# adolliou/euispice_coreg

Hardware: AMD Instinct MI355X
Metric: lag-points/sec (whole node) on 2048² grid, 60×60 CRVAL sweep; argmax-shift match (higher is better)
Workload: dtype f64; 1 GPU; headline: Carrington 'fa' 2048x2048 grid lon(200,300) lat(-20,20), 60x60 CRVAL lags arange(-30,30,1) arcsec, small 2048^2 HRIEUV-like, ref 3072^2 FSI-like, order 2, solar_r 1.004; lag_points=3600, parallelism=single GPU, no collective, resident=True, sweeps_in_flight=2, small_stored_f32=True, use_lds=True

## Files before the change

### euispice_coreg_amd/csrc/coreg_hip.hip

```cpp
#include <hip/hip_runtime.h>

#include <algorithm>
#include <chrono>
#include <cmath>
#include <cstdio>
#include <cstdlib>
#include <cstring>
#include <limits>
#include <condition_variable>
#include <map>
#include <memory>
#include <mutex>
#include <string>
#include <thread>
#include <functional>
#include <type_traits>
#include <utility>
#include <vector>

#include "fit.hpp"
#include "geometry.hpp"
#include "kernels.hpp"
#include <atomic>
#include "ricecomp.hpp"
#include "riceenc.hpp"

using namespace coreg;

#define COREG_VERSION "0.1.0"

#include "lag_plan.hpp"
#include "sweep_plan.hpp"
#include "host_owned.hpp"
#include "host_state.hpp"
#include "host_upload.hpp"
#include "host_smooth.hpp"
#include "host_plan.hpp"
#include "host_fix_launch.hpp"
#include "sweep_variant.hpp"
#include "host_sweep_launch.hpp"
#include "host_sweep_mi.hpp"
#include "host_fix_lists.hpp"
#include "host_sweep_io.hpp"
#include "host_context.hpp"
#include "pixels_plan.hpp"
#include "host_pixels.hpp"

coreg_handle::~coreg_handle() = default;

extern "C" {

const char* coreg_version(void) { return "coreg_hip " COREG_VERSION " (gfx950)"; }

int coreg_create(coreg_handle** out, int device) {
    if (!out) return COREG_EINVAL;
    *out = nullptr;
    int ndev = 0;
    hipError_t e = hipGetDeviceCount(&ndev);
    if (e != hipSuccess || ndev < 1) return COREG_EHIP;
    if (device < 0) {
        if (hipGetDevice(&device) != hipSuccess) device = 0;
    }
    if (device >= ndev) return COREG_EINVAL;
    coreg_handle* h = new (std::nothrow) coreg_handle();
    if (!h) return COREG_ENOMEM;
    h->device = device;
    if (hipSetDevice(device) != hipSuccess || hipStreamCreateWithFlags(&h->stream.s, hipStreamNonBlocking) != hipSuccess ||
        hipEventCreate(&h->ev_end[0].e) != hipSuccess ||
        hipEventCreate(&h->ev_end[1].e) != hipSuccess || hipEventRecord(h->ev_end[0], h->stream) != hipSuccess ||
        hipEventRecord(h->ev_end[1], h->stream) != hipSuccess ||
        h->pivots.reserve(2 * sizeof(double)) != hipSuccess ||
        hipMemsetAsync(h->pivots.p, 0, 2 * sizeof(double), h->stream) != hipSuccess) {
        coreg_destroy(h);
        return COREG_EHIP;
    }
    std::memset(&h->stats, 0, sizeof(h->stats));
    *out = h;
    return COREG_OK;
}

void coreg_destroy(coreg_handle* h) {
    if (!h) return;
    (void)hipSetDevice(h->device);
    if (h->up_thread.joinable()) {
        {
            std::unique_lock<std::mutex> lk(h->up_m);
            h->up_cv.wait(lk, [&] { return !h->up_busy && !h->up_has; });
            h->up_stop = true;
        }
        h->up_cv.notify_all();
        h->up_thread.join();
    }
    if (h->stream) (void)hipStreamSynchronize(h->stream);
    if (h->up_stream) (void)hipStreamSynchronize(h->up_stream);
    delete h;
}

const char* coreg_last_error(const coreg_handle* h) { return h ? h->err.c_str() : "null handle"; }

int coreg_set_stream(coreg_handle* h, void* hip_stream) {
    if (!h) return COREG_EINVAL;
    RETCHK(bind_device(h));
    RETCHK(collect_stats(h));
    HIPCHK(hipStreamSynchronize(h->stream));
    HIPCHK(h->stream.borrow((hipStream_t)hip_stream));
    return COREG_OK;
}

int coreg_synchronize(coreg_handle* h) {
    if (!h) return COREG_EINVAL;
    RETCHK(bind_device(h));
    HIPCHK(hipStreamSynchronize(h->stream));
    return COREG_OK;
}

int coreg_set_option(coreg_handle* h, const char* name, int64_t value) {
    if (!h || !name) return COREG_EINVAL;
    const std::string n(name);
    if (n == "use_lds") {
        h->opt_use_lds = value ? 1 : 0;
    } else if (n == "clean_path") {
        h->opt_clean_path = value ? 1 : 0;
    } else if (n == "tap_nan_filter") {
        if (value < 0 || value > 2) return fail(h, COREG_EINVAL, "tap_nan_filter must be 0, 1 or 2");
        h->opt_tap_nan_filter = value;
    } else if (n == "overlap_upload") {
        h->opt_overlap_upload = value ? 1 : 0;
    } else if (n == "async_upload") {
        h->opt_async_upload = value ? 1 : 0;
    } else if (n == "refine") {
        h->opt_refine = value ? 1 : 0;
    } else if (n == "refine_cond_log10") {
        if (value < -3 || value > 15) return fail(h, COREG_EINVAL, "refine_cond_log10 must be in [-3, 15]");
        h->opt_refine_cond_log10 = value;
    } else if (n == "refine_max") {
        if (value < 0 || value > 16) return fail(h, COREG_EINVAL, "refine_max must be in [0, 16]");
    } else if (n == "tile_w") {
        if (value != 0 && (value < 1 || value > kTilePts || (value & (value - 1)) != 0))
            return fail(h, COREG_EINVAL, "tile_w must be 0 or a power of two <= 1024");
        h->opt_tile_w = value;
    } else if (n == "n_groups") {
        if (value < 0) return fail(h, COREG_EINVAL, "n_groups must be >= 0");
        h->opt_n_groups = value;
    } else if (n == "sweep_wgs") {
        if (value < 0) return fail(h, COREG_EINVAL, "sweep_wgs must be >= 0");
        h->opt_sweep_wgs = value;
    } else if (n == "skew") {
        (void)value;
    } else if (n == "shard_world") {
        if (value < 1 || value > 64) return fail(h, COREG_EINVAL, "shard_world must be in [1, 64]");
        h->opt_shard_world = value;
        if (h->opt_shard_rank >= value) h->opt_shard_rank = 0;
    } else if (n == "combo_begin") {
        if (value < 0) return fail(h, COREG_EINVAL, "combo_begin must be >= 0");
        h->opt_combo_begin = value;
    } else if (n == "combo_end") {
        if (value < 0) return fail(h, COREG_EINVAL, "combo_end must be >= 0");
        h->opt_combo_end = value;
    } else if (n == "shard_rank") {
        if (value < 0 || value >= h->opt_shard_world) return fail(h, COREG_EINVAL, "shard_rank must be in [0, shard_world)");
        h->opt_shard_rank = value;
    } else if (n == "border_fix") {
        h->opt_border_fix = value ? 1 : 0;
    } else if (n == "tap_fix") {
        h->opt_tap_fix = value ? 1 : 0;
    } else if (n == "tap_cap") {
        if (value < 1 || value > (1 << 26)) return fail(h, COREG_EINVAL, "tap_cap must be in [1, 2^26]");
        h->opt_tap_cap = value;
    } else if (n == "pitch") {
        h->opt_pitch = value;
    } else if (n == "taper_frac") {
        if (value < -1 || value > 1000) return fail(h, COREG_EINVAL, "taper_frac must be in [-1, 1000]");
        h->opt_taper_frac = value;
    } else if (n == "taper_min") {
        if (value < 16 || value > 1024) return fail(h, COREG_EINVAL, "taper_min must be in [16, 1024]");
        h->opt_taper_min = value;
    } else if (n == "taper_rounds") {
        if (value < 1) return fail(h, COREG_EINVAL, "taper_rounds must be >= 1");
        h->opt_taper_rounds = value;
    } else if (n == "crop_reference") {
        h->opt_crop_reference = value ? 1 : 0;
    } else if (n == "tile_skip") {
        h->opt_tile_skip = value ? 1 : 0;
    } else if (n == "h_series") {
        h->opt_h_series = value ? 1 : 0;
    } else if (n == "h_incr") {
        h->opt_h_incr = value ? 1 : 0;
    } else if (n == "patch_w") {
        if (value < 0 || value > kBlock) return fail(h, COREG_EINVAL, "patch_w must be in [0, 256]");
        h->opt_patch_w = value;
    } else if (n == "mi_chunks") {
        if (value < 0 || value > kMiMaxChunks) return fail(h, COREG_EINVAL, "mi_chunks must be in [0, 64]");
        h->opt_mi_chunks = value;
    } else if (n == "lds_bytes") {
        if (value < 1024 || value > 159 * 1024) return fail(h, COREG_EINVAL, "lds_bytes must be in [1 KiB, 159 KiB]");
        h->opt_lds_bytes = value;
    } else {
        return fail(h, COREG_EINVAL, "unknown option: " + n);
    }
    return COREG_OK;
}

}

#include "abi_images.hpp"
#include "abi_sweeps.hpp"
#include "abi_host.hpp"
#include "abi_context.hpp"
#include "abi_pixels.hpp"


#include "multi.hpp"
```

### euispice_coreg_amd/csrc/host_plan.hpp

```cpp
#pragma once
namespace {

struct ComboRange {
    long long begin = 0, end = 0;
};
ComboRange take_combo_range(coreg_handle* h) {
    ComboRange r;
    r.begin = h->opt_combo_begin;
    r.end = h->opt_combo_end;
    h->opt_combo_begin = h->opt_combo_end = 0;
    return r;
}
int check_lags(coreg_handle* h, const coreg_lags* l, LagDims* d, int64_t begin, int64_t end, ComboRange combo = ComboRange()) {
    if (!l || !l->crval1 || !l->crval2 || !l->cdelt1 || !l->cdelt2 || !l->crota)
        return fail(h, COREG_EINVAL, "lags: null array");
    if (l->n_crval1 < 1 || l->n_crval2 < 1 || l->n_cdelt1 < 1 || l->n_cdelt2 < 1 || l->n_crota < 1)
        return fail(h, COREG_EINVAL, "lags: every axis needs at least one value");
    d->n1 = l->n_crval1;
    d->n2 = l->n_crval2;
    d->n3 = l->n_cdelt1;
    d->n4 = l->n_cdelt2;
    d->n5 = l->n_crota;
    d->nc = (long long)d->n3 * d->n4 * d->n5;
    d->c0 = 0;
    {
        const long long cb = combo.begin, ce = combo.end;
        if (cb != 0 || ce != 0) {
            if (cb < 0 || ce <= cb || ce > d->nc)
                return fail(h, COREG_EINVAL, "combo_begin/combo_end outside [0, n_cdelt1 * n_cdelt2 * n_crota]");
            d->c0 = cb;
            d->nc = ce - cb;
        }
    }
    if (begin < 0 || end > d->total() || begin > end)
        return fail(h, COREG_EINVAL, "lag_begin/lag_end outside [0, n_lags]");
    const double* ax[5] = {l->crval1, l->crval2, l->cdelt1, l->cdelt2, l->crota};
    const int32_t na[5] = {l->n_crval1, l->n_crval2, l->n_cdelt1, l->n_cdelt2, l->n_crota};
    for (int k = 0; k < 5; ++k)
        for (int32_t i = 0; i < na[k]; ++i)
            if (!std::isfinite(ax[k][i])) return fail(h, COREG_EINVAL, "lags: a non-finite value");
    return COREG_OK;
}

static int check_wcs(coreg_handle* h, const coreg_wcs2d* w, bool carrington_transform) {
    const char* why = wcs_problem(*w, carrington_transform);
    return why ? fail(h, COREG_EINVAL, why) : COREG_OK;
}
static int check_grid(coreg_handle* h, const coreg_carr_grid* g) {
    if (g->n_lon >= 1 && g->n_lat >= 1 && too_many(g->n_lon, g->n_lat))
        return fail(h, COREG_EINVAL, "Carrington grid: more than 2^31 - 1 points");
    const char* why = grid_problem(*g);
    return why ? fail(h, COREG_EINVAL, why) : COREG_OK;
}

int pick_groups(const coreg_handle* h, int n_batches, int n_tiles) {
    (void)n_tiles;
    return coreg::pick_groups(h->opt_shard_world, h->opt_n_groups, n_batches);
}

long long lds_window_elems(const coreg_handle* h);
SweepEnv sweep_env(coreg_handle* h) {
    SweepEnv e;
    e.sW = h->sW;
    e.sH = h->sH;
    e.gW = h->gW;
    e.gH = h->gH;
    e.border_fix = h->opt_border_fix != 0;
    e.tap_fix = h->opt_tap_fix != 0;
    e.use_lds = h->opt_use_lds != 0;
    e.h_series = h->opt_h_series != 0;
    e.tile_skip = h->opt_tile_skip != 0;
    e.lds_elems = lds_window_elems(h);
    e.tile_w = (int)h->opt_tile_w;
    e.patch_w = (int)h->opt_patch_w;
    e.shard_world = h->opt_shard_world;
    e.n_groups = h->opt_n_groups;
    e.pitch = h->opt_pitch;
    e.tabs = &h->tabs;
    e.caches = &h->wcslib;
    e.memo = &h->plan_memo;
    return e;
}

void pick_taper(const coreg_handle* h, int n_groups, int n_batches, int* tmin, int* tfrac) {
    *tmin = (int)h->opt_taper_min;
    if (h->opt_taper_frac >= 0) {
        *tfrac = (int)h->opt_taper_frac;
        return;
    }
    const double rounds = (double)n_groups * n_batches / 256.0;
    *tfrac = (rounds >= (double)h->opt_taper_rounds && n_groups >= 128 && h->opt_shard_world <= 1) ? 512 : 0;
}

template <int MODE>
int launch_precompute(coreg_handle* h, const PrecomputeArgs& a, int n_tiles, int n_groups, int n_batches) {
    EventPair* ev = next_event(h, h->ev_pre, h->ev_pre_used);
    if (!ev) return fail(h, COREG_EHIP, "hipEventCreate failed");
    int tmin, tfrac;
    pick_taper(h, n_groups, n_batches, &tmin, &tfrac);
    PrecomputeArgs b = a;
    b.prologue = h->pending_prologue;
    const bool with_prologue = b.prologue.src != nullptr;
    std::memset(&h->pending_prologue, 0, sizeof(h->pending_prologue));
    HIPCHK(hipEventRecord(ev->a, h->stream));
    if (h->ref_dtype == COREG_F32)
        hipLaunchKernelGGL((k_precompute<MODE, float>), dim3(n_tiles), dim3(256), 0, h->stream, b);
    else
        hipLaunchKernelGGL((k_precompute<MODE, double>), dim3(n_tiles), dim3(256), 0, h->stream, b);
    (void)with_prologue;
    hipLaunchKernelGGL(k_tile_list, dim3(1), dim3(1024), 0, h->stream, (const int*)a.tile_count, n_tiles, n_groups,
                       h->tile_list.as<int>(), h->tile_cum.as<int>(), h->group_first.as<int>(),
                       h->tile_info.as<long long>(), tmin, tfrac, (const double*)a.tile_bbox,
                       h->visit_rec.as<VisitRec>());
    ev->b_is_next_sweep = true;
    ev->next_sweep_index = h->ev_sweep_used;
    HIPCHK(hipGetLastError());
    return COREG_OK;
}

int reserve_tiles(coreg_handle* h, int n_tiles) {
    const size_t pts = (size_t)n_tiles * kTilePts + (size_t)(kPointGroups + 1) * kChunk;
    HIPCHK(h->pts.reserve(pts * sizeof(Pt)));
    HIPCHK(h->tile_count.reserve(n_tiles * sizeof(int)));
    HIPCHK(h->tile_list.reserve(n_tiles * sizeof(int)));
    HIPCHK(h->tile_cum.reserve((n_tiles + 1) * sizeof(int)));
    HIPCHK(h->group_first.reserve(2 * 1024 * sizeof(int) + 64));
    HIPCHK(h->tile_info.reserve(8 * sizeof(long long)));
    HIPCHK(h->tile_bbox.reserve((size_t)n_tiles * 4 * sizeof(double)));
    HIPCHK(h->visit_rec.reserve(((size_t)n_tiles + 1) * sizeof(VisitRec)));
    return COREG_OK;
}

int setup_precompute(coreg_handle* h, const Plan& plan, int method, PrecomputeArgs* a, int* n_tiles) {
    std::memset(a, 0, sizeof(*a));
    a->tile_w = plan.tile_w;
    a->tile_h = kTilePts / plan.tile_w;
    a->tiles_x = (h->gW + a->tile_w - 1) / a->tile_w;
    a->tiles_y = (h->gH + a->tile_h - 1) / a->tile_h;
    *n_tiles = a->tiles_x * a->tiles_y;
    RETCHK(reserve_tiles(h, *n_tiles));
    a->ref = h->ref.p;
    a->gw = h->gW;
    a->gh = h->gH;
    a->pivot_a = h->pivots.as<double>();
    a->pts = h->pts.as<Pt>();
    a->tile_count = h->tile_count.as<int>();
    a->tile_bbox = h->tile_bbox.as<double>();
    a->residus = method != COREG_METHOD_CORRELATION ? 1 : 0;
    return COREG_OK;
}

}
```

### euispice_coreg_amd/csrc/host_state.hpp

```cpp
#pragma once
namespace {

enum SrcKind {
    SRC_HOST = 0,
    SRC_PINNED = 1,
    SRC_DEVICE = 2,
    SRC_TILED = 3,
};

struct PixFmt {
    int bitpix = 0;
    bool f32 = false;
    double bscale = 1.0, bzero = 0.0;
    bool raw() const { return bitpix != 0; }
    bool scaled() const { return bscale != 1.0 || bzero != 0.0; }
    size_t elem() const { return raw() ? (size_t)(bitpix < 0 ? -bitpix : bitpix) / 8 : (f32 ? 4 : 8); }
    bool swap_only() const { return bitpix == -32 && !scaled(); }
    static PixFmt native(bool is_f32) {
        PixFmt f;
        f.f32 = is_f32;
        return f;
    }
};

constexpr int kMaxDevices = 64;
std::mutex g_attr_mutex;

struct EventPair {
    Event a, b;
    bool b_is_next_sweep = false;
    size_t next_sweep_index = 0;
};

}

struct KeptTapLists {
    DevBuf all;
};
struct TapFix {
    TapFixArgs args = {};
    int segs = 0;
    int mode = 0;
    long long count = 0;
};
struct FixLaunch {
    std::vector<BorderFixArgs> border;
    std::vector<ParityFixArgs> parity;
    TapFix tap;
    std::shared_ptr<KeptTapLists> kept;
    bool small_f32 = true;
    bool empty() const { return border.empty() && parity.empty() && tap.segs == 0; }
};

struct ContextState;
struct PixelsState;

struct coreg_handle {
    int device = 0;
    Stream stream;
    std::string err;

    std::unique_ptr<ContextState> ctx;
    std::unique_ptr<PixelsState> pix;
    ~coreg_handle();

    DevBuf small;
    int sW = 0, sH = 0;
    bool small_f32 = false;
    DevBuf ref;
    int gW = 0, gH = 0;
    int ref_dtype = -1;
    DevBuf pivots, red_sum, red_cnt;
    DevBuf t_sin_lon, t_cos_lon, t_cos_lat, t_sin_lat, t_lon_deg, t_dx;
    coreg_diffrot rot_ref = {}, rot_small = {};
    bool has_rot_ref = false, has_rot_small = false;
    DevBuf sm_num, sm_den, sm_out;
    std::vector<double> ref_smooth_y, ref_smooth_x;
    CarrTables tabs;
    std::vector<double> tabs_key;
    bool tabs_uploaded = false;
    PinBuf pin_img[2];
    Event ev_img[2];
    int pin_img_next = 0;
    DevBuf pts, tile_count, tile_list, tile_cum, group_first, tile_info, tile_bbox;
    DevBuf visit_rec;
    DevBuf rf_fix_slab;
    DevBuf counters;
    DevBuf lane_params, out_index, partials, out_dev, tmp_img;
    DevBuf sweep_queue;
    int n_cus = 0;
    struct SweepResidency {
        const void* fn;
        size_t lds_bytes;
        int per_cu;
    };
    std::vector<SweepResidency> sweep_residency;
    int64_t opt_sweep_wgs = 0;
    DevBuf counts;
    long long counts_n = -1;
    DevBuf up_f64, up_flag;
    DevBuf up_raw;
    DevBuf rice_blob, rice_rand, dec_img;
    PrologueArgs pending_prologue = {};
    DevBuf bbox_buf;
    Stream aux_stream;
    Stream up_stream;
    Event ev_small, ev_main;
    bool small_pending = false;
    DevBuf red_sum_up, red_cnt_up;
    int64_t opt_overlap_upload = 1;
    int64_t opt_tap_nan_filter = 2;
    int64_t opt_async_upload = 0;
    std::thread up_thread;
    std::mutex up_m;
    std::condition_variable up_cv;
    std::function<hipError_t()> up_job;
    bool up_has = false, up_stop = false, up_busy = false;
    hipError_t up_rc = hipSuccess;
    PinBuf pin_small[2];
    Event ev_pin_small[2];
    int pin_small_next = 0;
    WcslibCaches wcslib;
    DevBuf border_flags, fix_partial;
    DevBuf border_dev;
    PinBuf pin_border;
    int64_t opt_border_fix = 1;
    int64_t opt_tap_fix = 1, opt_tap_cap = 1 << 24;
    DevBuf tap_count, tap_segq, tap_list, tap_skip, tap_seg_slot, tap_seg_begin, tap_pixel, tap_xw, tap_yw;
    long long tap_last[3] = {0, 0, 0};
    int last_variant[7] = {-1, 0, 0, 0, 0, 0, 0};
    int64_t opt_shard_world = 1, opt_shard_rank = 0;
    int64_t opt_combo_begin = 0, opt_combo_end = 0;
    DevBuf sums;
    long long sums_slots = 0;
    struct PendingFinalize {
        long long slot_off, n_slots, lag_begin;
        int residus;
        RefineArgs refine;
        std::function<int(coreg_handle*)> replay_precompute;
        FixLaunch fixes;
    };
    std::function<int(coreg_handle*)> last_precompute;
    PlanMemo plan_memo;
    DevBuf rf_flags, rf_pivots, rf_list, rf_head, rf_partial;
    std::vector<PendingFinalize> pending_fin;
    DevBuf fin_outidx;
    long long pending_n_out = 0;
    std::vector<double> mi_edges_small, mi_edges_large;
    DevBuf mi_hist;
    size_t mi_lds[6] = {0, 0, 0, 0, 0, 0};
    int64_t opt_mi_chunks = 0;

    int64_t opt_crop_reference = 1;
    int64_t opt_taper_min = 128, opt_taper_frac = -1, opt_taper_rounds = 6;
    int64_t opt_use_lds = 1, opt_clean_path = 1, opt_refine = 1, opt_refine_cond_log10 = 5, opt_tile_w = 0, opt_n_groups = 0, opt_lds_bytes = (159 * 1024 * kPointGroups) / 4, opt_patch_w = 0, opt_h_series = 1, opt_h_incr = 1, opt_tile_skip = 1, opt_pitch = -1;

    coreg_stats stats;
    bool stats_pending = false;
    PinBuf pin_info;
    std::vector<EventPair> ev_sweep, ev_pre;
    size_t ev_sweep_used = 0, ev_pre_used = 0;
    hipEvent_t ev_t1 = nullptr;
    Event ev_end[2];
    PinBuf pin_plan[2];
    int plan_slot = 0;
    bool plan_open = false;
};
```

### euispice_coreg_amd/csrc/kernels_prepare.hpp

```cpp
#pragma once
namespace coreg {
template <typename T>
__global__ void __launch_bounds__(256) k_sum_finite(const T* __restrict__ v, long long n, double* part_sum,
                                                    long long* part_cnt) {
    __shared__ double ss[256];
    __shared__ long long sc[256];
    double s = 0.0;
    long long c = 0;
    for (long long i = (long long)blockIdx.x * 256 + threadIdx.x; i < n; i += (long long)gridDim.x * 256) {
        const double x = (double)v[i];
        if (isfinite(x)) {
            s += x;
            ++c;
        }
    }
    ss[threadIdx.x] = s;
    sc[threadIdx.x] = c;
    __syncthreads();
    for (int o = 128; o > 0; o >>= 1) {
        if ((int)threadIdx.x < o) {
            ss[threadIdx.x] += ss[threadIdx.x + o];
            sc[threadIdx.x] += sc[threadIdx.x + o];
        }
        __syncthreads();
    }
    if (threadIdx.x == 0) {
        part_sum[blockIdx.x] = ss[0];
        part_cnt[blockIdx.x] = sc[0];
    }
}
__global__ void k_mean_final(const double* part_sum, const long long* part_cnt, int n, double* mean_out) {
    if (threadIdx.x == 0 && blockIdx.x == 0) {
        double s = 0.0;
        long long c = 0;
        for (int i = 0; i < n; ++i) {
            s += part_sum[i];
            c += part_cnt[i];
        }
        mean_out[0] = c > 0 ? s / (double)c : 0.0;
    }
}

__global__ void __launch_bounds__(256) k_f32_exact(const double* __restrict__ v, long long n, int* flag) {
    int bad = 0;
    for (long long i = (long long)blockIdx.x * 256 + threadIdx.x; i < n; i += (long long)gridDim.x * 256) {
        const double x = v[i];
        if (x == x && (double)(float)x != x) bad = 1;
    }
    if (bad) atomicOr(flag, 1);
}
__global__ void __launch_bounds__(256) k_f64_to_f32(const double* __restrict__ v, long long n, float* __restrict__ out) {
    for (long long i = (long long)blockIdx.x * 256 + threadIdx.x; i < n; i += (long long)gridDim.x * 256)
        out[i] = (float)v[i];
}

__global__ void __launch_bounds__(256) k_fits_swap32(unsigned int* __restrict__ v, long long n) {
    for (long long i = (long long)blockIdx.x * 256 + threadIdx.x; i < n; i += (long long)gridDim.x * 256)
        v[i] = __builtin_bswap32(v[i]);
}
__global__ void __launch_bounds__(256) k_fits_to_f64(const void* __restrict__ raw, int bitpix, int scaled, double bscale,
                                                     double bzero, long long n, double* __restrict__ out) {
#pragma clang fp contract(off)
    for (long long i = (long long)blockIdx.x * 256 + threadIdx.x; i < n; i += (long long)gridDim.x * 256) {
        double x;
        switch (bitpix) {
            case 8: x = (double)((const unsigned char*)raw)[i]; break;
            case 16: x = (double)(short)__builtin_bswap16(((const unsigned short*)raw)[i]); break;
            case 32: x = (double)(int)__builtin_bswap32(((const unsigned int*)raw)[i]); break;
            case 64: x = (double)(long long)__builtin_bswap64(((const unsigned long long*)raw)[i]); break;
            case -32: x = (double)__uint_as_float(__builtin_bswap32(((const unsigned int*)raw)[i])); break;
            default: x = __longlong_as_double((long long)__builtin_bswap64(((const unsigned long long*)raw)[i])); break;
        }
        if (scaled) x = x * bscale + bzero;
        out[i] = x;
    }
}

template <typename T>
__global__ void __launch_bounds__(256) k_threshold(T* __restrict__ v, long long n, int has_min, double vmin, int has_max,
                                                   double vmax) {
    for (long long i = (long long)blockIdx.x * 256 + threadIdx.x; i < n; i += (long long)gridDim.x * 256) {
        const double x = fabs((double)v[i]);
        if ((has_min && x < vmin) || (has_max && x > vmax)) v[i] = (T)__builtin_nan("");
    }
}

__global__ void k_fill(double* p, long long n, double v) {
    const long long i = (long long)blockIdx.x * blockDim.x + threadIdx.x;
    if (i < n) p[i] = v;
}

struct ResampleArgs {
    const void* img;
    int W, H;
    int gw, gh;
    CarrDev carr;
    double x0, y0;
    H9 hom;
    void* out;
    int order_rt;
    Crop crop;
    double* bbox;
    LaunchU car_fwd, car_inv;
};
template <int MODE>
__device__ __forceinline__ bool resample_coord(const ResampleArgs& a, long long idx, double& nx, double& ny) {
    const int i = (int)(idx % a.gw), j = (int)(idx / a.gw);
    bool ok = true;
    if (MODE == MODE_TRANSLATE) {
        double t0, t1;
        ok = carr_term(a.carr, i, j, t0, t1);
        nx = a.x0 + t0;
        ny = a.y0 + t1;
    } else if (MODE == MODE_CAR) {
        const double phi = fma(a.car_fwd.m00, (double)i, fma(a.car_fwd.m01, (double)j, a.car_fwd.b0));
        const double theta = fma(a.car_fwd.m10, (double)i, fma(a.car_fwd.m11, (double)j, a.car_fwd.b1));
        apply_car(a.hom, a.car_inv, phi, theta, nx, ny);
    } else {
        apply_h(a.hom, (double)i, (double)j, nx, ny);
    }
    if (!ok) nx = __builtin_nan("");
    return (nx >= 0.0) & (nx <= (double)(a.W - 1)) & (ny >= 0.0) & (ny <= (double)(a.H - 1));
}
template <int MODE>
__global__ void __launch_bounds__(256) k_resample_bbox(const ResampleArgs a) {
    __shared__ double red[4][4];
    const double inf = __builtin_inf();
    double mnx = inf, mxx = -inf, mny = inf, mxy = -inf;
    const long long n = (long long)a.gw * a.gh;
    for (long long idx = (long long)blockIdx.x * 256 + threadIdx.x; idx < n; idx += (long long)gridDim.x * 256) {
        double nx, ny;
        if (resample_coord<MODE>(a, idx, nx, ny)) {
            mnx = fmin(mnx, nx);
            mxx = fmax(mxx, nx);
            mny = fmin(mny, ny);
            mxy = fmax(mxy, ny);
        }
    }
    for (int o = 32; o > 0; o >>= 1) {
        mnx = fmin(mnx, __shfl_xor(mnx, o));
        mxx = fmax(mxx, __shfl_xor(mxx, o));
        mny = fmin(mny, __shfl_xor(mny, o));
        mxy = fmax(mxy, __shfl_xor(mxy, o));
    }
    const int lane = threadIdx.x & 63, wave = threadIdx.x >> 6;
    if (lane == 0) {
        red[wave][0] = mnx;
        red[wave][1] = mxx;
        red[wave][2] = mny;
        red[wave][3] = mxy;
    }
    __syncthreads();
    if (threadIdx.x == 0) {
// ... 39 lines not shown
    for (long long i = i0; i < p.n_outidx; i += stride) p.dst_outidx[i] = src_idx[i];
    const double nan = __builtin_nan("");
    for (long long i = i0; i < p.n_out; i += stride) p.out[i] = nan;
    if (p.counts)
        for (long long i = i0; i < p.n_out; i += stride) p.counts[i] = nan;
}

struct PrecomputeArgs {
    PrologueArgs prologue;
    const void* ref;
    int gw, gh;
    int tile_w, tile_h;
    int tiles_x, tiles_y;
    CarrDev carr;
    LaunchU car_fwd;
    double f0lo, f0hi, f1lo, f1hi;
    int residus;
    int tile_skip;
    double lip_x, lip_y;
    double dlon, dlat;
    const double* pivot_a;
    Pt* pts;
    int* tile_count;
    double* tile_bbox;
};
template <int MODE, typename TA>
__global__ void __launch_bounds__(256) k_precompute(const PrecomputeArgs a) {
    __shared__ int wave_cnt[4];
    __shared__ double red[4][4];
    run_prologue(a.prologue);
    const int tile = blockIdx.x;
    const int tx = tile % a.tiles_x, ty = tile / a.tiles_x;
    const int lane = threadIdx.x & 63, wave = threadIdx.x >> 6;
    const double pivot = a.pivot_a[0];
    const double inf = __builtin_inf();
    if (MODE == MODE_TRANSLATE && a.tile_skip) {
        __shared__ int s_skip;
        const int i0 = tx * a.tile_w, j0 = ty * a.tile_h;
        const int i1 = min(i0 + a.tile_w, a.gw) - 1, j1 = min(j0 + a.tile_h, a.gh) - 1;
        if (threadIdx.x == 0) {
            const int ic = (i0 + i1) / 2, jc = (j0 + j1) / 2;
            double t0, t1;
            carr_term(a.carr, ic, jc, t0, t1);
            const double ang = (double)max(ic - i0, i1 - ic) * a.dlon + (double)max(jc - j0, j1 - jc) * a.dlat;
            const double m0 = a.lip_x * ang + 1.0, m1 = a.lip_y * ang + 1.0;
            s_skip = (t0 + m0 < a.f0lo) || (t0 - m0 > a.f0hi) || (t1 + m1 < a.f1lo) || (t1 - m1 > a.f1hi);
        }
        __syncthreads();
        if (s_skip) {
            if (threadIdx.x == 0) a.tile_count[tile] = 0;
            return;
        }
    }
    double mn0 = inf, mx0 = -inf, mn1 = inf, mx1 = -inf;
    int base_pos = 0;
    const size_t tbase = (size_t)tile * kTilePts;
    for (int r = 0; r < kTilePts / 256; ++r) {
        const int k = r * 256 + threadIdx.x;
        const int gi = tx * a.tile_w + (k % a.tile_w);
        const int gj = ty * a.tile_h + (k / a.tile_w);
        bool valid = (gi < a.gw) & (gj < a.gh);
        double b0 = 0.0, b1 = 0.0, av = 0.0;
        if (valid) {
            av = (double)((const TA*)a.ref)[(size_t)gj * a.gw + gi];
            if (MODE == MODE_TRANSLATE) {
                valid = carr_term(a.carr, gi, gj, b0, b1);
            } else if (MODE == MODE_CAR) {
                b0 = fma(a.car_fwd.m00, (double)gi, fma(a.car_fwd.m01, (double)gj, a.car_fwd.b0));
                b1 = fma(a.car_fwd.m10, (double)gi, fma(a.car_fwd.m11, (double)gj, a.car_fwd.b1));
            } else {
                b0 = (double)gi;
                b1 = (double)gj;
            }
            valid = valid & isfinite(av) & (b0 >= a.f0lo) & (b0 <= a.f0hi) & (b1 >= a.f1lo) & (b1 <= a.f1hi);
        }
        const unsigned long long bal = __ballot(valid);
        const int rank = __popcll(bal & ((1ull << lane) - 1ull));
        if (lane == 0) wave_cnt[wave] = __popcll(bal);
        __syncthreads();
        int off = base_pos;
        for (int w = 0; w < wave; ++w) off += wave_cnt[w];
        const int tot = wave_cnt[0] + wave_cnt[1] + wave_cnt[2] + wave_cnt[3];
        if (valid) {
            Pt pt;
            pt.b0 = b0;
            pt.b1 = b1;
            pt.a = a.residus ? av : av - pivot;
            pt.pad = a.residus ? 1.0 / sqrt(av) : 0.0;
            if (MODE == MODE_CAR) {
                double sp, cp, st, ct;
                sincos(b0, &sp, &cp);
                sincos(b1, &st, &ct);
                pt.b0 = ct * cp;
                pt.b1 = ct * sp;
                pt.pad = st;
            }
            a.pts[tbase + off + rank] = pt;
            mn0 = fmin(mn0, b0);
            mx0 = fmax(mx0, b0);
            mn1 = fmin(mn1, b1);
            mx1 = fmax(mx1, b1);
        }
        base_pos += tot;
        __syncthreads();
    }
    if (MODE != MODE_CAR && !a.residus) {
        static_assert(kChunk >= 3, "run flag + the two chunk sums live in the pads of the chunk's first three points");
        Pt* tp = a.pts + tbase;
        for (int c = threadIdx.x; c < base_pos / kChunk; c += 256) {
            double sa = tp[c * kChunk].a, saa = sa * sa;
            bool run = MODE == MODE_HOMOGRAPHY || MODE == MODE_HOMOGRAPHY_SERIES;
#pragma unroll
            for (int k = 1; k < kChunk; ++k) {
                const double v = tp[c * kChunk + k].a;
                sa += v;
                saa = fma(v, v, saa);
                run = run && tp[c * kChunk + k].b0 == tp[c * kChunk].b0 + (double)k && tp[c * kChunk + k].b1 == tp[c * kChunk].b1;
            }
            tp[c * kChunk].pad = run ? 1.0 : 0.0;
            tp[c * kChunk + 1].pad = sa;
            tp[c * kChunk + 2].pad = saa;
        }
    }
    for (int o = 32; o > 0; o >>= 1) {
        mn0 = fmin(mn0, __shfl_xor(mn0, o));
        mx0 = fmax(mx0, __shfl_xor(mx0, o));
        mn1 = fmin(mn1, __shfl_xor(mn1, o));
        mx1 = fmax(mx1, __shfl_xor(mx1, o));
    }
    if (lane == 0) {
        red[wave][0] = mn0;
        red[wave][1] = mx0;
        red[wave][2] = mn1;
        red[wave][3] = mx1;
    }
    __syncthreads();
    if (threadIdx.x == 0) {
        a.tile_count[tile] = base_pos;
        double* bb = a.tile_bbox + (size_t)tile * 4;
        bb[0] = fmin(fmin(red[0][0], red[1][0]), fmin(red[2][0], red[3][0]));
        bb[1] = fmax(fmax(red[0][1], red[1][1]), fmax(red[2][1], red[3][1]));
        bb[2] = fmin(fmin(red[0][2], red[1][2]), fmin(red[2][2], red[3][2]));
        bb[3] = fmax(fmax(red[0][3], red[1][3]), fmax(red[2][3], red[3][3]));
    }
}

constexpr int kUnitPts = kChunk * kPointGroups;
struct alignas(64) VisitRec {
    int tile_cum, tile, count, pad;
    double bbox[4];
    double fill[2];
};
static_assert(sizeof(VisitRec) == 64, "one record per 64-byte line");
__host__ __device__ inline long long group_start(int g, long long total, int n_groups, int taper_min, int taper_frac) {
    if (taper_frac <= 0) return (long long)g * total / n_groups;
    const int g0 = n_groups - (int)((long long)n_groups * taper_frac / 1024);
    const int nt = n_groups - 1 - g0;
    if (nt <= 0) return (long long)g * total / n_groups;
    const double m = (double)taper_min / 1024.0;
    auto cum = [&](int k) -> double {
        if (k <= g0) return (double)k;
        const double j = (double)(k - g0);
        return (double)g0 + j - (1.0 - m) * j * (j - 1.0) / (2.0 * (double)nt);
    };
    if (g >= n_groups) return total;
    const long long s0 = (long long)(cum(g) / cum(n_groups) * (double)total);
    return s0 < 0 ? 0 : (s0 > total ? total : s0);
}
__global__ void __launch_bounds__(1024) k_tile_list(const int* __restrict__ tile_count, int n_tiles, int n_groups,
                                                    int* tile_list, int* tile_cum, int* group_first, long long* info,
                                                    int taper_min, int taper_frac,
                                                    const double* __restrict__ tile_bbox, VisitRec* visit_rec) {
    __shared__ int wcnt[16];
    __shared__ int wunits[16];
    __shared__ long long wpts[16];
    __shared__ int s_base, s_units;
    __shared__ long long s_pts;
    const int lane = threadIdx.x & 63, wave = threadIdx.x >> 6;
    if (threadIdx.x == 0) {
        s_base = 0;
        s_units = 0;
        s_pts = 0;
    }
    __syncthreads();
    for (int t0 = 0; t0 < n_tiles; t0 += 1024) {
        const int t = t0 + threadIdx.x;
        const int c = t < n_tiles ? tile_count[t] : 0;
        const bool nz = c > 0;
        const int units = (c + kUnitPts - 1) / kUnitPts;
        const unsigned long long bal = __ballot(nz);
        const int rank = __popcll(bal & ((1ull << lane) - 1ull));
        long long pts = c;
        int uincl = units;
        for (int o = 1; o < 64; o <<= 1) {
            const int v = __shfl_up(uincl, o);
            if (lane >= o) uincl += v;
        }
        for (int o = 32; o > 0; o >>= 1) pts += __shfl_xor(pts, o);
        if (lane == 63) wunits[wave] = uincl;
        if (lane == 0) {
            wcnt[wave] = __popcll(bal);
            wpts[wave] = pts;
        }
        __syncthreads();
        int off = s_base, uoff = s_units;
        for (int w = 0; w < wave; ++w) {
            off += wcnt[w];
            uoff += wunits[w];
        }
        if (nz) {
            tile_list[off + rank] = t;
            tile_cum[off + rank] = uoff + uincl - units;
            VisitRec r;
            r.tile_cum = uoff + uincl - units;
            r.tile = t;
            r.count = c;
            r.pad = 0;
#pragma unroll
            for (int k = 0; k < 4; ++k) r.bbox[k] = tile_bbox[(size_t)t * 4 + k];
            r.fill[0] = r.fill[1] = 0.0;
            visit_rec[off + rank] = r;
        }
        __syncthreads();
        if (threadIdx.x == 0) {
            int tot = 0, tu = 0;
            long long tp = 0;
            for (int w = 0; w < 16; ++w) {
                tot += wcnt[w];
                tu += wunits[w];
                tp += wpts[w];
            }
            s_base += tot;
            s_units += tu;
            s_pts += tp;
        }
        __syncthreads();
    }
    const int n_list = s_base, total = s_units;
    if (threadIdx.x == 0) {
        tile_cum[n_list] = total;
        VisitRec r = {};
        r.tile_cum = total;
        visit_rec[n_list] = r;
        info[0] = n_list;
        info[1] = s_pts;
        info[2] = total;
        info[3] = info[4] = info[5] = info[6] = 0;
    }
    __syncthreads();
    for (int g = threadIdx.x; g <= n_groups; g += 1024) {
        const long long start = group_start(g, total, n_groups, taper_min, taper_frac);
        group_first[1024 + g] = (int)start;
        int lo = 0, hi = n_list;
        while (lo < hi) {
            const int mid = (lo + hi + 1) >> 1;
            if (mid <= n_list && (long long)tile_cum[mid] <= start) lo = mid;
            else hi = mid - 1;
        }
        group_first[g] = lo;
    }
}

}
```

### euispice_coreg_amd/csrc/kernels_sweep.hpp

```cpp
#pragma once
namespace coreg {
struct SweepArgs {
    const void* img;
    int W, H;
    const Pt* pts;
    const int* tile_count;
    const int* tile_list;
    const int* tile_cum;
    const int* group_first;
    long long* tile_info;
    const double* tile_bbox;
    const VisitRec* visit_rec;
    const double* lane_params;
    long long n_slots;
    int n_batches;
    int n_groups;
    int group_lo;
    double* partials;
    unsigned* queue;
    int items8;
    const double* pivots;
    int use_lds;
    int clean_path;
    int lds_elems;
// ... 514 lines not shown
                            xn = fma(hv.h[0], x, fma(hv.h[1], y, hv.h[2]));
                            yn = fma(hv.h[3], x, fma(hv.h[4], y, hv.h[5]));
                            ww = MODE == MODE_HOMOGRAPHY_SERIES ? fma(hv.h[6], x, hv.h[7] * y)
                                                                : fma(hv.h[6], x, fma(hv.h[7], y, hv.h[8]));
                        } else {
                            xn += hv.h[0];
                            yn += hv.h[3];
                            ww += hv.h[6];
                        }
                        double ux, uy;
                        if (MODE == MODE_HOMOGRAPHY_SERIES) {
                            const double qq = fma(ww, ww, -ww);
                            ux = fma(xn, qq, xn);
                            uy = fma(yn, qq, yn);
                        } else {
                            double r = __builtin_amdgcn_rcp(ww);
                            r = fma(r, fma(-ww, r, 1.0), r);
                            ux = xn * r;
                            uy = yn * r;
                        }
                        point_lag<MODE, ORDER, TS, LDS, ROUND, RESID, INTERIOR, PITCH, CLEAN, true>(
                            acc, win, img, pitch, ox, oy, W, H, wmax, hmax, px0, py0, pxw, pyw, hv, cu, ux, uy,
                            spt_f64(cur, 2), spt_f64(cur, 3), pivot_b);
                        if constexpr (CLEAN) {
                            if (k == 1) acc.a += spt_f64(cur, 3);
                            if (k == 2) acc.aa += spt_f64(cur, 3);
                            if (k == kChunk - 1) acc.n += kChunk;
                        }
                        spt_wait(nxt);
                        cur = nxt;
                    }
                }
            }
            if (pg == n_full % kPointGroups) {
                for (int p = n_full * kChunk; p < p_end; ++p) {
                    Pt pt;
                    load_pt_uniform(pts + p, pt);
                    point_lag<MODE, ORDER, TS, LDS, ROUND, RESID, INTERIOR, PITCH>(acc, win, img, pitch, ox, oy, W, H, wmax,
                                                                                   hmax, px0, py0, pxw, pyw, hm, cu, pt.b0,
                                                                                   pt.b1, pt.a, pt.pad, pivot_b);
                }
            }
            return;
        }
    }
    {
        int c = p_begin / kChunk + pg;
        if (c < n_full) {
            H9 hml = hm;
            double& anchor = MODE == MODE_TRANSLATE ? (INTERIOR && LDS ? pxw : px0) : hml.h[MODE == MODE_CAR ? 0 : 7];
            SPt cur = spt_load(pts + c * kChunk, anchor);
            spt_wait(cur);
            for (; c < n_full; c += kPointGroups) {
                const Pt* __restrict__ q = pts + c * kChunk;
#pragma unroll
                for (int k = 0; k < kChunk; ++k) {
                    SPt nxt = spt_load(k + 1 < kChunk ? q + k + 1 : q + kPointGroups * kChunk, anchor);
                    point_lag<MODE, ORDER, TS, LDS, ROUND, RESID, INTERIOR, PITCH, CLEAN>(
                        acc, win, img, pitch, ox, oy, W, H, wmax, hmax, px0, py0, pxw, pyw, hml, cu, spt_f64(cur, 0),
                        spt_f64(cur, 1), spt_f64(cur, 2), spt_f64(cur, 3), pivot_b);
                    if constexpr (CLEAN) {
                        if (k == 1) acc.a += spt_f64(cur, 3);
                        if (k == 2) acc.aa += spt_f64(cur, 3);
                        if (k == kChunk - 1) acc.n += kChunk;
                    }
                    spt_wait(nxt);
                    cur = nxt;
                }
            }
        }
    }
#else
    for (int c = p_begin / kChunk + pg; c < n_full; c += kPointGroups) {
        const Pt* __restrict__ q = pts + c * kChunk;
        Pt pt[kChunk];
#pragma unroll
        for (int k = 0; k < kChunk; ++k) load_pt_uniform(q + k, pt[k]);
#pragma unroll
        for (int k = 0; k < kChunk; ++k)
            point_lag<MODE, ORDER, TS, LDS, ROUND, RESID, INTERIOR, PITCH, CLEAN>(acc, win, img, pitch, ox, oy, W, H, wmax,
                                                                                  hmax, px0, py0, pxw, pyw, hm, cu, pt[k].b0,
                                                                                  pt[k].b1, pt[k].a, pt[k].pad, pivot_b);
        if constexpr (CLEAN) {
            acc.n += kChunk;
            acc.a += pt[1].pad;
            acc.aa += pt[2].pad;
        }
    }
#endif
    if (pg == n_full % kPointGroups) {
        for (int p = n_full * kChunk; p < p_end; ++p) {
            Pt pt;
            load_pt_uniform(pts + p, pt);
            point_lag<MODE, ORDER, TS, LDS, ROUND, RESID, INTERIOR, PITCH>(acc, win, img, pitch, ox, oy, W, H, wmax, hmax,
                                                                           px0, py0, pxw, pyw, hm, cu, pt.b0, pt.b1, pt.a,
                                                                           pt.pad, pivot_b);
        }
    }
}

template <int MODE, int ORDER, typename TS, bool ROUND, bool RESID, int PITCH = 0>
__global__ void __launch_bounds__(kSweepThreads) k_sweep(const SweepArgs a) {
    extern __shared__ __align__(16) unsigned char lds_raw[];
    double* lds = (double*)lds_raw;
    constexpr int kWaves = kSweepThreads / 64;
    constexpr int kLagWaves = kBlock / 64;
    __shared__ double wred2[2][kLagWaves][4];
    __shared__ int wdirty[2][kWaves];
    constexpr bool kCleanPath = MODE != MODE_CAR && !RESID && ORDER != ORDER_RT && !(ROUND && sizeof(TS) == 8);
    int n_vis = 0, n_vis_lds = 0, n_vis_int = 0, n_vis_clean = 0;

    __shared__ int next_q[2];
    const int slot8 = blockIdx.x & 7;
    int q = blockIdx.x >> 3;
    int item_par = 0;

    const int lane = threadIdx.x & 63, wave = threadIdx.x >> 6;
    const int pg = __builtin_amdgcn_readfirstlane(wave % kPointGroups);
    const int lw = __builtin_amdgcn_readfirstlane(wave / kPointGroups);
    const int ls = 64 * lw + lane;

    const TS* __restrict__ img = (const TS*)a.img;
    const int W = a.W, H = a.H;
    const double inf = __builtin_inf();
    const double pivot_b = a.pivots[1];
#if defined(__HIP_DEVICE_COMPILE__)
    const unsigned win = (unsigned)(uintptr_t)(__attribute__((address_space(3))) unsigned char*)lds_raw;
#else
    const unsigned win = 0;
#endif

    while (q < a.items8) {
    const int batch = q % a.n_batches;
    const int group = a.group_lo + (q / a.n_batches) * 8 + slot8;
    const long long slot = (long long)batch * kBlock + ls;
    int visit = 0;

    double px0 = 0.0, py0 = 0.0;
    H9 hm;
#pragma unroll
    for (int k = 0; k < 9; ++k) hm.h[k] = 0.0;
    if (MODE == MODE_TRANSLATE) {
        px0 = a.lane_params[slot];
        py0 = a.lane_params[a.n_slots + slot];
    } else {
#pragma unroll
        for (int k = 0; k < 9; ++k) hm.h[k] = a.lane_params[(long long)k * a.n_slots + slot];
    }

    const bool pad_lane = MODE == MODE_TRANSLATE ? (px0 != px0) : (hm.h[8] != hm.h[8]);

    Acc acc = {0, 0.0, 0.0, 0.0, 0.0, 0.0};

    const int u_lo = a.group_first[1024 + group];
    const int u_hi = a.group_first[1024 + group + 1];

    constexpr bool kLagBox = MODE == MODE_TRANSLATE && COREG_VISIT_LAGBOX;
    double lx0 = 0.0, lx1 = 0.0, ly0 = 0.0, ly1 = 0.0;
    if constexpr (kLagBox) {
        lx0 = lx1 = px0;
        ly0 = ly1 = py0;
        for (int o = 32; o > 0; o >>= 1) {
            lx0 = fmin(lx0, __shfl_xor(lx0, o));
            lx1 = fmax(lx1, __shfl_xor(lx1, o));
            ly0 = fmin(ly0, __shfl_xor(ly0, o));
            ly1 = fmax(ly1, __shfl_xor(ly1, o));
        }
        if (lane == 0 && pg == 0) {
            wred2[0][lw][0] = lx0;
            wred2[0][lw][1] = lx1;
            wred2[0][lw][2] = ly0;
            wred2[0][lw][3] = ly1;
        }
        __syncthreads();
        lx0 = fmin(fmin(wred2[0][0][0], wred2[0][1][0]), fmin(wred2[0][2][0], wred2[0][3][0]));
        lx1 = fmax(fmax(wred2[0][0][1], wred2[0][1][1]), fmax(wred2[0][2][1], wred2[0][3][1]));
        ly0 = fmin(fmin(wred2[0][0][2], wred2[0][1][2]), fmin(wred2[0][2][2], wred2[0][3][2]));
        ly1 = fmax(fmax(wred2[0][0][3], wred2[0][1][3]), fmax(wred2[0][2][3], wred2[0][3][3]));
    }

    int tl = a.group_first[group];
    unsigned park = 0;
    {
        Visit first;
        load_visit_uniform(a.visit_rec + tl, first);
        park = park_visit(first, park);
    }
    for (; u_lo < u_hi; ++tl) {
        Visit cur;
        unpark_visit(park, cur);
        const int ubase = cur.ubase;
        if (ubase >= u_hi) break;
        Visit nxt;
        load_visit_uniform(a.visit_rec + tl + 1, nxt);
        const int tile = cur.tile;
        const int cnt = cur.cnt;
        const int p_begin = max(u_lo - ubase, 0) * kUnitPts;
        const int p_end = min((u_hi - ubase) * kUnitPts, cnt);
        if (p_begin >= p_end) {
            park = park_visit(nxt, park);
            continue;
        }
        const double bx0 = cur.bx0, bx1 = cur.bx1, by0 = cur.by0, by1 = cur.by1;

        double mnx, mxx, mny, mxy;
        if constexpr (kLagBox) {
            mnx = bx0 + lx0;
            mxx = bx1 + lx1;
            mny = by0 + ly0;
            mxy = by1 + ly1;
        } else if (MODE == MODE_TRANSLATE) {
            mnx = bx0 + px0;
            mxx = bx1 + px0;
            mny = by0 + py0;
            mxy = by1 + py0;
        } else {
            mnx = inf; mxx = -inf; mny = inf; mxy = -inf;
#pragma unroll
            for (int c = 0; c < 4; ++c) {
                double cx, cy;
                apply_map<MODE>(hm, a.car_inv, (c & 1) ? bx1 : bx0, (c & 2) ? by1 : by0, cx, cy);
                mnx = fmin(mnx, cx);
                mxx = fmax(mxx, cx);
                mny = fmin(mny, cy);
                mxy = fmax(mxy, cy);
            }
            if (MODE == MODE_CAR) {
                const double margin = car_tile_margin(a.car_inv.box_c, fmax(fabs(by0), fabs(by1)) + a.car_inv.pole_sep);
                mnx -= margin;
                mxx += margin;
                mny -= margin;
                mxy += margin;
            }
        }
        int* wdirt = wdirty[visit & 1];
        if constexpr (!kLagBox) {
            for (int o = 32; o > 0; o >>= 1) {
                mnx = fmin(mnx, __shfl_xor(mnx, o));
                mxx = fmax(mxx, __shfl_xor(mxx, o));
                mny = fmin(mny, __shfl_xor(mny, o));
                mxy = fmax(mxy, __shfl_xor(mxy, o));
            }
            double(*wred)[4] = wred2[visit & 1];
            if (lane == 0 && pg == 0) {
                wred[lw][0] = mnx;
                wred[lw][1] = mxx;
                wred[lw][2] = mny;
                wred[lw][3] = mxy;
            }
            __syncthreads();
            mnx = fmin(fmin(wred[0][0], wred[1][0]), fmin(wred[2][0], wred[3][0]));
            mxx = fmax(fmax(wred[0][1], wred[1][1]), fmax(wred[2][1], wred[3][1]));
            mny = fmin(fmin(wred[0][2], wred[1][2]), fmin(wred[2][2], wred[3][2]));
            mxy = fmax(fmax(wred[0][3], wred[1][3]), fmax(wred[2][3], wred[3][3]));
        }
        ++visit;
        if (!(mxx >= 0.0) || !(mnx <= (double)(W - 1)) || !(mxy >= 0.0) || !(mny <= (double)(H - 1))) {
            park = park_visit(nxt, park);
            continue;
        }
        if constexpr (kLagBox) __syncthreads();
        constexpr double kClear = 1e-9;
        const bool interior = (mnx >= kClear) & (mxx <= (double)(W - 1) - kClear) & (mny >= kClear) &
                              (mxy <= (double)(H - 1) - kClear);
        constexpr bool kWide = ORDER == ORDER_RT || ORDER > 2;
        const int ord = ORDER == ORDER_RT ? a.car_inv.order_rt : ORDER;
        const int ap_lo = kWide ? ord / 2 + 1 : 1;
        const int ap_hi = kWide ? ord - ord / 2 + 1 : 2;
        const int ox = max((int)floor(fmax(mnx, 0.0)) - ap_lo, kWide ? -ap_lo : -1);
        const int oy = max((int)floor(fmax(mny, 0.0)) - ap_lo, kWide ? -ap_lo : -1);
        const int ex = min((int)floor(fmin(mxx, (double)(W - 1))) + ap_hi, kWide ? W - 1 + ap_hi : W);
        const int ey = min((int)floor(fmin(mxy, (double)(H - 1))) + ap_hi, kWide ? H - 1 + ap_hi : H);
        const int ww = ex - ox + 1, wh = ey - oy + 1;
        int pitch = PITCH > 0 ? PITCH : (ww | 1);
        if (PITCH == 0) {
            const int r = pitch & 31;
            const int up = r < 5 ? 5 - r : ((r > 11 && r < 21) ? 21 - r : (r > 27 ? 37 - r : 0));
            if ((long long)(pitch + up) * wh <= (long long)a.lds_elems) pitch += up;
        }
        const long long need = (long long)pitch * wh;
        const bool in_lds = a.use_lds && (need <= (long long)a.lds_elems) && (PITCH == 0 || ww <= PITCH);

        const Pt* __restrict__ pts = a.pts + (size_t)tile * kTilePts;

        bool swept = false;
        ++n_vis;
        {
          if (in_lds) {
            swept = true;
            ++n_vis_lds;
#ifndef COREG_STAGE_ROWS
#define COREG_STAGE_ROWS 8
#endif
#ifndef COREG_STAGE_COLS
#define COREG_STAGE_COLS 1
#endif
            constexpr int kStage = COREG_STAGE_ROWS, kCols = COREG_STAGE_COLS;
            const double scale = ORDER == 2 ? 0.25 : 1.0;
            constexpr bool kFmaStage = ORDER == 2 && !ROUND && COREG_VISIT_FMA;
            const double npivot4 = -0.25 * pivot_b;
            const int wave_u = __builtin_amdgcn_readfirstlane(wave);
            double poison = 0.0;
            for (int r0 = wave_u; r0 < wh; r0 += kWaves * kStage) {
                for (int c0 = 0; c0 < ww; c0 += 64 * kCols) {
                    int gx[kCols];
#pragma unroll
                    for (int j = 0; j < kCols; ++j) {
                        const int c = c0 + 64 * j + lane;
                        gx[j] = kWide ? mirror_far(ox + min(c, ww - 1), W) : mirror_idx(ox + min(c, ww - 1), W);
                    }
                    TS v[kStage][kCols];
#pragma unroll
                    for (int k = 0; k < kStage; ++k) {
                        const int r = min(r0 + k * kWaves, wh - 1);
                        const int gy = kWide ? mirror_far(oy + r, H) : mirror_idx(oy + r, H);
                        const TS* __restrict__ row = img + (size_t)gy * W;
#pragma unroll
                        for (int j = 0; j < kCols; ++j) v[k][j] = row[gx[j]];
                    }
#pragma unroll
                    for (int j = 0; j < kCols; ++j) {
                        const int c = c0 + 64 * j + lane;
                        if (c < ww) {
#pragma unroll
                            for (int k = 0; k < kStage; ++k) {
                                const int r = r0 + k * kWaves;
                                if (r < wh) {
                                    const double e = (kFmaStage ? fma((double)v[k][j], 0.25, npivot4)
                                                                : (ROUND ? (double)v[k][j] : (double)v[k][j] - pivot_b) * scale);
                                    lds[r * pitch + c] = e;
                                    if (kCleanPath) poison = fma(e, 0.0, poison);
                                }
                            }
                        }
// ... 97 lines not shown
```

Baseline: 1.275 million lag-points/s.

## Snap group shares to tile boundaries and deal groups by size

Group start offsets are now snapped to the nearest tile boundary, so a work group no longer starts partway through a tile and splits its visits. A size-ranked deal permutation, ordered largest first and serpentine across blocks of eight, maps workgroup index to share, so the biggest shares launch early and the tail is more even. Both are on by default when there are many groups and rounds. The cost is a sort-like ranking pass in k_tile_list, and the snapping can make group sizes less even.

New measurement: 1.286 million lag-points/s (median of 6 runs). About the same (+0.8%).

```diff
diff --git a/euispice_coreg_amd/csrc/coreg_hip.hip b/euispice_coreg_amd/csrc/coreg_hip.hip
--- a/euispice_coreg_amd/csrc/coreg_hip.hip
+++ b/euispice_coreg_amd/csrc/coreg_hip.hip
@@ -145,6 +145,9 @@
     } else if (n == "sweep_wgs") {
         if (value < 0) return fail(h, COREG_EINVAL, "sweep_wgs must be >= 0");
         h->opt_sweep_wgs = value;
+    } else if (n == "share_snap") {
+        if (value < -1 || value > 2) return fail(h, COREG_EINVAL, "share_snap must be -1, 0, 1 or 2");
+        h->opt_share_snap = value;
     } else if (n == "skew") {
         (void)value;
     } else if (n == "shard_world") {
diff --git a/euispice_coreg_amd/csrc/host_plan.hpp b/euispice_coreg_amd/csrc/host_plan.hpp
--- a/euispice_coreg_amd/csrc/host_plan.hpp
+++ b/euispice_coreg_amd/csrc/host_plan.hpp
@@ -88,8 +88,11 @@
         *tfrac = (int)h->opt_taper_frac;
         return;
     }
-    const double rounds = (double)n_groups * n_batches / 256.0;
-    *tfrac = (rounds >= (double)h->opt_taper_rounds && n_groups >= 128 && h->opt_shard_world <= 1) ? 512 : 0;
+    *tfrac = (many_rounds_many_groups(n_groups, n_batches, h->opt_taper_rounds) && h->opt_shard_world <= 1) ? 512 : 0;
+}
+
+int pick_share_snap(const coreg_handle* h, int n_groups, int n_batches) {
+    return resolve_share_snap(h->opt_share_snap, h->opt_shard_world, n_groups, n_batches, h->opt_taper_rounds);
 }
 
 template <int MODE>
@@ -110,7 +113,8 @@
     (void)with_prologue;
     hipLaunchKernelGGL(k_tile_list, dim3(1), dim3(1024), 0, h->stream, (const int*)a.tile_count, n_tiles, n_groups,
                        h->tile_list.as<int>(), h->tile_cum.as<int>(), h->group_first.as<int>(),
-                       h->tile_info.as<long long>(), tmin, tfrac, (const double*)a.tile_bbox,
+                       h->tile_info.as<long long>(), tmin, tfrac,
+                       pick_share_snap(h, n_groups, n_batches), (const double*)a.tile_bbox,
                        h->visit_rec.as<VisitRec>());
     ev->b_is_next_sweep = true;
     ev->next_sweep_index = h->ev_sweep_used;
@@ -124,7 +128,7 @@
     HIPCHK(h->tile_count.reserve(n_tiles * sizeof(int)));
     HIPCHK(h->tile_list.reserve(n_tiles * sizeof(int)));
     HIPCHK(h->tile_cum.reserve((n_tiles + 1) * sizeof(int)));
-    HIPCHK(h->group_first.reserve(2 * 1024 * sizeof(int) + 64));
+    HIPCHK(h->group_first.reserve(3 * 1024 * sizeof(int) + 64));
     HIPCHK(h->tile_info.reserve(8 * sizeof(long long)));
     HIPCHK(h->tile_bbox.reserve((size_t)n_tiles * 4 * sizeof(double)));
     HIPCHK(h->visit_rec.reserve(((size_t)n_tiles + 1) * sizeof(VisitRec)));
diff --git a/euispice_coreg_amd/csrc/host_state.hpp b/euispice_coreg_amd/csrc/host_state.hpp
--- a/euispice_coreg_amd/csrc/host_state.hpp
+++ b/euispice_coreg_amd/csrc/host_state.hpp
@@ -95,6 +95,7 @@
         int per_cu;
     };
     std::vector<SweepResidency> sweep_residency;
+    int64_t opt_share_snap = -1;
     int64_t opt_sweep_wgs = 0;
     DevBuf counts;
     long long counts_n = -1;
diff --git a/euispice_coreg_amd/csrc/kernels_prepare.hpp b/euispice_coreg_amd/csrc/kernels_prepare.hpp
--- a/euispice_coreg_amd/csrc/kernels_prepare.hpp
+++ b/euispice_coreg_amd/csrc/kernels_prepare.hpp
@@ -1,4 +1,5 @@
 #pragma once
+#include "tile_shares.hpp"
 namespace coreg {
 template <typename T>
 __global__ void __launch_bounds__(256) k_sum_finite(const T* __restrict__ v, long long n, double* part_sum,
@@ -344,30 +345,17 @@
     double fill[2];
 };
 static_assert(sizeof(VisitRec) == 64, "one record per 64-byte line");
-__host__ __device__ inline long long group_start(int g, long long total, int n_groups, int taper_min, int taper_frac) {
-    if (taper_frac <= 0) return (long long)g * total / n_groups;
-    const int g0 = n_groups - (int)((long long)n_groups * taper_frac / 1024);
-    const int nt = n_groups - 1 - g0;
-    if (nt <= 0) return (long long)g * total / n_groups;
-    const double m = (double)taper_min / 1024.0;
-    auto cum = [&](int k) -> double {
-        if (k <= g0) return (double)k;
-        const double j = (double)(k - g0);
-        return (double)g0 + j - (1.0 - m) * j * (j - 1.0) / (2.0 * (double)nt);
-    };
-    if (g >= n_groups) return total;
-    const long long s0 = (long long)(cum(g) / cum(n_groups) * (double)total);
-    return s0 < 0 ? 0 : (s0 > total ? total : s0);
-}
 __global__ void __launch_bounds__(1024) k_tile_list(const int* __restrict__ tile_count, int n_tiles, int n_groups,
                                                     int* tile_list, int* tile_cum, int* group_first, long long* info,
-                                                    int taper_min, int taper_frac,
+                                                    int taper_min, int taper_frac, int share_snap,
                                                     const double* __restrict__ tile_bbox, VisitRec* visit_rec) {
     __shared__ int wcnt[16];
     __shared__ int wunits[16];
     __shared__ long long wpts[16];
     __shared__ int s_base, s_units;
     __shared__ long long s_pts;
+    __shared__ int s_start[1024];
+    __shared__ int s_size[1024], s_rank[1024];
     const int lane = threadIdx.x & 63, wave = threadIdx.x >> 6;
     if (threadIdx.x == 0) {
         s_base = 0;
@@ -440,17 +428,31 @@
         info[3] = info[4] = info[5] = info[6] = 0;
     }
     __syncthreads();
+    const bool snap = share_snap_active(share_snap, n_list, n_groups, 1);
     for (int g = threadIdx.x; g <= n_groups; g += 1024) {
-        const long long start = group_start(g, total, n_groups, taper_min, taper_frac);
-        group_first[1024 + g] = (int)start;
-        int lo = 0, hi = n_list;
-        while (lo < hi) {
-            const int mid = (lo + hi + 1) >> 1;
-            if (mid <= n_list && (long long)tile_cum[mid] <= start) lo = mid;
-            else hi = mid - 1;
-        }
-        group_first[g] = lo;
-    }
-}
-
-}
+        const ShareStart s = share_start(g, tile_cum, n_list, n_groups, taper_min, taper_frac, snap);
+        group_first[1024 + g] = s.unit;
+        group_first[g] = s.entry;
+        s_start[g] = s.unit;
+    }
+    __syncthreads();
+    const bool deal = share_deal_active(share_snap, snap, n_groups);
+    if (deal) {
+        for (int g = threadIdx.x; g < n_groups; g += 1024) {
+            s_size[g] = s_start[g + 1] - s_start[g];
+            s_rank[g] = 0;
+        }
+        __syncthreads();
+        const int parts = max(1, 1024 / n_groups), len = (n_groups + parts - 1) / parts;
+        for (int i = threadIdx.x; i < n_groups * parts; i += 1024) {
+            const int g = i % n_groups, h0 = (i / n_groups) * len;
+            const int r = share_rank_part(s_size, h0, min(h0 + len, n_groups), g);
+            if (r) atomicAdd(&s_rank[g], r);
+        }
+        __syncthreads();
+    }
+    for (int g = threadIdx.x; g < n_groups; g += 1024)
+        group_first[2048 + (deal ? deal_position(s_rank[g]) : g)] = g;
+}
+
+}
diff --git a/euispice_coreg_amd/csrc/kernels_sweep.hpp b/euispice_coreg_amd/csrc/kernels_sweep.hpp
--- a/euispice_coreg_amd/csrc/kernels_sweep.hpp
+++ b/euispice_coreg_amd/csrc/kernels_sweep.hpp
@@ -690,8 +690,9 @@
 
     Acc acc = {0, 0.0, 0.0, 0.0, 0.0, 0.0};
 
-    const int u_lo = a.group_first[1024 + group];
-    const int u_hi = a.group_first[1024 + group + 1];
+    const int share = a.group_first[2048 + group];
+    const int u_lo = a.group_first[1024 + share];
+    const int u_hi = a.group_first[1024 + share + 1];
 
     constexpr bool kLagBox = MODE == MODE_TRANSLATE && COREG_VISIT_LAGBOX;
     double lx0 = 0.0, lx1 = 0.0, ly0 = 0.0, ly1 = 0.0;
@@ -717,7 +718,7 @@
         ly1 = fmax(fmax(wred2[0][0][3], wred2[0][1][3]), fmax(wred2[0][2][3], wred2[0][3][3]));
     }
 
-    int tl = a.group_first[group];
+    int tl = a.group_first[share];
     unsigned park = 0;
     {
         Visit first;
diff --git a/euispice_coreg_amd/csrc/tile_shares.hpp b/euispice_coreg_amd/csrc/tile_shares.hpp
--- /dev/null
+++ b/euispice_coreg_amd/csrc/tile_shares.hpp
@@ -0,0 +1,89 @@
+#pragma once
+
+#if defined(__HIPCC__) || defined(__CUDACC__)
+#define COREG_SHARES_HD __host__ __device__
+#else
+#define COREG_SHARES_HD
+#endif
+
+namespace coreg {
+
+COREG_SHARES_HD inline long long group_start(int g, long long total, int n_groups, int taper_min, int taper_frac) {
+    if (taper_frac <= 0) return (long long)g * total / n_groups;
+    const int g0 = n_groups - (int)((long long)n_groups * taper_frac / 1024);
+    const int nt = n_groups - 1 - g0;
+    if (nt <= 0) return (long long)g * total / n_groups;
+    const double m = (double)taper_min / 1024.0;
+    auto cum = [&](int k) -> double {
+        if (k <= g0) return (double)k;
+        const double j = (double)(k - g0);
+        return (double)g0 + j - (1.0 - m) * j * (j - 1.0) / (2.0 * (double)nt);
+    };
+    if (g >= n_groups) return total;
+    const long long s0 = (long long)(cum(g) / cum(n_groups) * (double)total);
+    return s0 < 0 ? 0 : (s0 > total ? total : s0);
+}
+
+COREG_SHARES_HD inline bool many_rounds_many_groups(int n_groups, int n_batches, long long min_rounds) {
+    return (double)n_groups * n_batches / 256.0 >= (double)min_rounds && n_groups >= 128;
+}
+COREG_SHARES_HD inline int resolve_share_snap(long long opt, long long shard_world, int n_groups, int n_batches,
+                                              long long min_rounds) {
+    if (shard_world > 1) return 0;
+    if (opt >= 0) return (int)opt;
+    return many_rounds_many_groups(n_groups, n_batches, min_rounds) ? 1 : 0;
+}
+
+COREG_SHARES_HD inline bool share_snap_active(long long share_snap, int n_list, int n_groups, long long shard_world) {
+    return share_snap != 0 && shard_world <= 1 && (long long)n_list >= 2ll * (long long)n_groups;
+}
+
+COREG_SHARES_HD inline int share_entry(const int* tile_cum, int n_list, long long u) {
+    int lo = 0, hi = n_list;
+    while (lo < hi) {
+        const int mid = (lo + hi + 1) >> 1;
+        if ((long long)tile_cum[mid] <= u) lo = mid;
+        else hi = mid - 1;
+    }
+    return lo;
+}
+
+struct ShareStart {
+    int entry;
+    int unit;
+};
+
+COREG_SHARES_HD inline ShareStart share_start(int g, const int* tile_cum, int n_list, int n_groups, int taper_min,
+                                              int taper_frac, bool snap) {
+    const long long total = tile_cum[n_list];
+    const long long ideal = group_start(g, total, n_groups, taper_min, taper_frac);
+    int k = share_entry(tile_cum, n_list, ideal);
+    if (!snap) return ShareStart{k, (int)ideal};
+    if (k < n_list && ideal - (long long)tile_cum[k] > (long long)tile_cum[k + 1] - ideal) ++k;
+    return ShareStart{k, tile_cum[k]};
+}
+
+COREG_SHARES_HD inline int share_rank_part(const int* units, int h0, int h1, int g) {
+    const int u = units[g];
+    int r = 0;
+#if defined(__HIP_DEVICE_COMPILE__)
+#pragma unroll 8
+#endif
+    for (int h = h0; h < h1; ++h) {
+        const int v = units[h];
+        r += (v > u) | ((v == u) & (h < g));
+    }
+    return r;
+}
+COREG_SHARES_HD inline int share_rank(const int* units, int n_groups, int g) {
+    return share_rank_part(units, 0, n_groups, g);
+}
+COREG_SHARES_HD inline int deal_position(int r) {
+    const int p = r >> 3, s = r & 7;
+    return 8 * p + ((p & 1) ? 7 - s : s);
+}
+COREG_SHARES_HD inline bool share_deal_active(long long share_snap, bool snap_active, int n_groups) {
+    return snap_active && share_snap == 1 && (n_groups & 7) == 0;
+}
+
+}
diff --git a/profiles/tile_shares_predict.py b/profiles/tile_shares_predict.py
--- /dev/null
+++ b/profiles/tile_shares_predict.py
@@ -0,0 +1,55 @@
+#!/usr/bin/env python3
+import os
+import subprocess
+import sys
+import tempfile
+
+import numpy as np
+
+ROOT = os.path.dirname(os.path.dirname(os.path.abspath(__file__)))
+sys.path.insert(0, ROOT)
+from euispice_coreg_amd import synthetic
+from oracle import coreg_oracle as O
+from profiles.lds_bank_sim import lag_origins
+
+GRID, LON, LAT, SOLAR_R = 2048, [200.0, 300.0], [-20.0, 20.0], 1.004
+TILE_PTS, N_BATCHES = 1024, 15
+
+
+def pick_groups(n_batches):
+    g = (4096 + n_batches - 1) // n_batches
+    return max(8, min(256, (g + 7) // 8 * 8))
+
+
+def main():
+    small, hs, large, hl, truth = synthetic.make_scene()
+    hs = dict(hs)
+    O.check_and_create_pcij_matrix(hs)
+    lag = np.arange(-30, 30, 1.0)
+    X0, Y0 = lag_origins(hs, lag, lag)
+    nx, ny = O.carrington_coords(hs, SOLAR_R, [GRID, GRID], LON, LAT)
+    x00, y00 = lag_origins(hs, np.array([0.0]), np.array([0.0]))
+    T0, T1 = nx - x00[0, 0], ny - y00[0, 0]
+    H, W = small.shape
+    keep = (np.isfinite(T0) & np.isfinite(T1) & (T0 >= -X0.max()) & (T0 <= W - 1 - X0.min()) & (T1 >= -Y0.max()) &
+            (T1 <= H - 1 - Y0.min()))
+    n_groups = pick_groups(N_BATCHES)
+    rounds = n_groups * N_BATCHES / 256.0
+    tfrac = 512 if rounds >= 6 and n_groups >= 128 else 0
+    print(f"# headline: {GRID}^2 grid, {keep.sum()} of {keep.size} points kept, {n_groups} groups x {N_BATCHES} batches, "
+          f"taper 128/{tfrac}")
+    with tempfile.TemporaryDirectory() as tmp:
+        exe = os.path.join(tmp, "tile_shares_rules")
+        subprocess.run(["g++", "-std=c++17", "-O1", os.path.join(ROOT, "tests", "native", "tile_shares_rules.cpp"), "-o", exe],
+                       check=True)
+        for tw in [int(a) for a in sys.argv[1:]] or [32]:
+            th = TILE_PTS // tw
+            counts = keep.reshape(GRID // th, th, GRID // tw, tw).sum(axis=(1, 3)).ravel()
+            print(f"# tile {tw} x {th}")
+            r = subprocess.run([exe, "count", str(n_groups), str(N_BATCHES), "128", str(tfrac)],
+                               input=" ".join(str(int(c)) for c in counts), capture_output=True, text=True, check=True)
+            print(r.stdout, end="")
+
+
+if __name__ == "__main__":
+    main()
```
